# XPU-Forces/mojo_opset

Hardware: AMD Instinct MI355X
Metric: MojoPagedDecodeGQA tokens/s (Llama-3-8B shape, bf16, 1/8 MI355X) (higher is better)
Workload: dtype bf16; 1 GPU; MojoPagedDecodeGQA bf16, B=64, 32q/8kv, head_dim=128, page=16, ctx=4096 uniform, AABB, random block tables (BASELINE configs[1]); per_gpu_batch=64, parallelism=replicas x1 (no collective on this path)

## Files before the change

### mojo_opset_amd/csrc/paged_decode_gqa.hip

```cpp
#include <math.h>
#include <stdlib.h>

#include "common.h"

namespace mojo {

constexpr int DEC_LPT = 16;
constexpr int DEC_TPL = 64 / DEC_LPT;
constexpr int DEC_LOADS = 4;
constexpr int DEC_TILE = DEC_TPL * DEC_LOADS;

template <typename T> struct pack8;
template <> struct pack8<bf16_t> {
  typedef bf16x8 vec;
  typedef bf16x2 pair;
  static __device__ __forceinline__ float dot2(pair a, pair b, float c) {
    return __builtin_amdgcn_fdot2_f32_bf16(a, b, c, false);
  }
};
template <> struct pack8<f16_t> {
  typedef f16x8 vec;
  typedef f16x2 pair;
  static __device__ __forceinline__ float dot2(pair a, pair b, float c) { return __builtin_amdgcn_fdot2(a, b, c, false); }
};
// ... 494 lines not shown
    chunk = ceil_div(len, s2);
    if (chunk < 128) chunk = 128;
    chunk = ceil_div(chunk, DEC_TILE) * DEC_TILE;
  }
  return static_cast<int>(chunk);
}

static int64_t decode_max_len(int64_t page, int64_t max_pages, int64_t hint) {
  const int64_t cap = page * max_pages;
  return (hint > 0 && hint < cap) ? hint : cap;
}

static int64_t decode_swa_cap(int64_t max_len, int64_t local_window, int64_t global_window) {
  int64_t span = global_window > 0 ? ceil_div(global_window, DEC_TILE) * DEC_TILE : 0;
  if (local_window >= 0) span += local_window + DEC_TILE;
  return span < max_len ? span : max_len;
}

static bool decode_use_mfma(int64_t G, int64_t head_dim, int64_t page) {
  const bool pow2 = page > 0 && (page & (page - 1)) == 0;
  if (!pow2 || page < 16 || (head_dim != 64 && head_dim != 128) || G > 16) return false;
  const long long e = MOJO_SWITCH("MOJO_HIP_DECODE_MFMA", -1);
  if (e == 0) return false;
  if (e == 1) return true;
  return G >= 4 || head_dim == 64 || (G != 1 && G != 2);
}

struct DecodeGeom {
  int64_t batch = 0, q_heads = 0, kv_heads = 0, head_dim = 0, page = 0, max_pages = 0, len_hint = 0;
  int64_t local_window = -1, global_window = 0;
  bool kv8 = false;
};

struct DecodePlan {
  bool swa = false;
  bool mfma = false;
  int64_t capacity = 0;
  int64_t max_len = 0;
  int chunk_tokens = 0, n_chunks = 0, fuse_group = 0;
  int hshift = 0, grid_kv_heads = 0, G = 0;
  int64_t slots = 0;
  int64_t bytes = 0;
  int64_t query_bytes = 0;
};

static DecodePlan decode_plan(const DecodeGeom& g) {
  DecodePlan p;
  p.swa = g.local_window >= 0 || g.global_window > 0;
  if (g.batch <= 0 || g.kv_heads <= 0 || g.q_heads <= 0) return p;
  p.capacity = decode_max_len(g.page, g.max_pages, g.len_hint);
  p.max_len = p.swa ? decode_swa_cap(p.capacity, g.local_window, g.global_window) : p.capacity;
  const int64_t heads = g.q_heads / g.kv_heads;
  auto form = [&](int hshift, DecodePlan& f) {
    f.hshift = hshift;
    f.grid_kv_heads = static_cast<int>(g.kv_heads << hshift);
    f.G = static_cast<int>(heads >> hshift);
    f.mfma = !g.kv8 && decode_use_mfma(f.G, g.head_dim, g.page);
    const bool grouped = f.mfma && MOJO_SWITCH("MOJO_HIP_DECODE_GROUPED", 1) != 0 && MOJO_SWITCH("MOJO_HIP_DECODE_FUSE", 1) != 0;
    f.chunk_tokens = decode_chunk_tokens(g.batch, f.grid_kv_heads, p.max_len, grouped);
    f.n_chunks = static_cast<int>(ceil_div(p.max_len > 0 ? p.max_len : 1, f.chunk_tokens));
    f.fuse_group = grouped && f.n_chunks > 8 ? 8 : 0;
    f.slots = g.batch * g.kv_heads * f.n_chunks * heads;
  };
  const bool can_halve = !p.swa && !g.kv8 && heads == 8;
  int hshift = 0;
#ifdef MOJO_HIP_BUILD_EXPERIMENTS
  if (can_halve && MOJO_SWITCH("MOJO_HIP_DECODE_G8_HALVES", 0) == 1) hshift = 1;
#endif
  form(hshift, p);
  const int64_t slot_bytes = (g.head_dim + 2) * static_cast<int64_t>(sizeof(float));
  p.bytes = p.slots * slot_bytes;
  int64_t most = p.slots;
  if (can_halve) {
    DecodePlan other;
    form(1 - hshift, other);
    if (other.slots > most) most = other.slots;
  }
  p.query_bytes = most * slot_bytes + 256;
  return p;
}

template <typename T, bool NT, int MODE, bool SWA>
static void launch_decode_mfma(const DecodeArgs& a, dim3 grid, dim3 block, int G, hipStream_t s) {
  const size_t waves = block.x / 64;
  const size_t lds = (MODE != DEC_SPLIT ? waves * G * (a.dim + 2) * sizeof(float) : 0) + waves * 4096;
  static std::atomic<uint64_t> attr_set{0};
  if (first_call_on_device(attr_set)) {
    (void)hipFuncSetAttribute(reinterpret_cast<const void*>(&decode_mfma_kernel<T, 4, NT, MODE, SWA>), hipFuncAttributeMaxDynamicSharedMemorySize, 160 * 1024);
    (void)hipFuncSetAttribute(reinterpret_cast<const void*>(&decode_mfma_kernel<T, 2, NT, MODE, SWA>), hipFuncAttributeMaxDynamicSharedMemorySize, 160 * 1024);
  }
  if (a.dim == 128) hipLaunchKernelGGL((decode_mfma_kernel<T, 4, NT, MODE, SWA>), grid, block, lds, s, a, G);
  else hipLaunchKernelGGL((decode_mfma_kernel<T, 2, NT, MODE, SWA>), grid, block, lds, s, a, G);
}

template <typename T, bool NT, bool SWA>
static int launch_decode_nt(const DecodeArgs& a, const DecodePlan& p, hipStream_t s) {
  const int64_t batch = a.batch;
  const int G = p.G;
  const bool no_fuse = MOJO_SWITCH("MOJO_HIP_DECODE_FUSE", 1) == 0;
  const bool no_pair = MOJO_SWITCH("MOJO_HIP_DECODE_PAIR", 1) == 0;
  const char* nt_tag = NT ? "nt" : "cached";
  const char* swa_tag = SWA ? ":swa" : "";
  if (p.mfma) {
    if (!SWA && a.n_chunks == 4 && batch >= 2 && batch <= 64 && !no_fuse && !no_pair) {
      launch_decode_mfma<T, NT, DEC_PAIRED, false>(a, dim3(1, static_cast<unsigned>(((batch + 1) / 2) * a.hkv)), dim3(512), G, s);
      MOJO_CHECK_LAUNCH("paged_decode_gqa(mfma, paired)");
      note_launch("decode_mfma:paired:%s%s", nt_tag, swa_tag);
      return MOJO_OK;
    }
    if (a.n_chunks <= 8 && !no_fuse) {
      launch_decode_mfma<T, NT, DEC_FUSED, SWA>(a, dim3(1, static_cast<unsigned>(batch * a.hkv)), dim3(static_cast<unsigned>(64 * a.n_chunks)), G, s);
      MOJO_CHECK_LAUNCH("paged_decode_gqa(mfma, fused)");
      note_launch("decode_mfma:fused:%s%s", nt_tag, swa_tag);
      return MOJO_OK;
    }
    if (a.fuse_group > 0 && !no_fuse) {
      const unsigned n_sub = static_cast<unsigned>((a.n_chunks + a.fuse_group - 1) / a.fuse_group);
      launch_decode_mfma<T, NT, DEC_FUSED, SWA>(a, dim3(n_sub, static_cast<unsigned>(batch * a.hkv)), dim3(static_cast<unsigned>(64 * a.fuse_group)), G, s);
      MOJO_CHECK_LAUNCH("paged_decode_gqa(mfma, grouped)");
      hipLaunchKernelGGL((decode_merge_kernel<T, SWA>), dim3(static_cast<unsigned>(batch * a.hkv), G), dim3(256), 0, s, a, G);
      MOJO_CHECK_LAUNCH("paged_decode_gqa(merge)");
      note_launch("decode_mfma:grouped+merge:%s%s", nt_tag, swa_tag);
      return MOJO_OK;
    }
    launch_decode_mfma<T, NT, DEC_SPLIT, SWA>(a, dim3(static_cast<unsigned>(a.n_chunks), static_cast<unsigned>(batch * a.hkv)), dim3(64), G, s);
    MOJO_CHECK_LAUNCH("paged_decode_gqa(mfma, split)");
    hipLaunchKernelGGL((decode_merge_kernel<T, SWA>), dim3(static_cast<unsigned>(batch * a.hkv), G), dim3(256), 0, s, a, G);
    MOJO_CHECK_LAUNCH("paged_decode_gqa(merge)");
    note_launch("decode_mfma:split+merge:%s%s", nt_tag, swa_tag);
    return MOJO_OK;
  }
  if (!SWA && a.n_chunks == 4 && batch >= 2 && batch <= 64 && a.dim % 4 == 0 && !no_fuse && !no_pair) {
    dim3 grid(1, static_cast<unsigned>(((batch + 1) / 2) * a.hkv));
    const size_t lds = static_cast<size_t>(8) * G * (a.dim + 2) * sizeof(float) + (G >= 8 ? static_cast<size_t>(8) * G * DEC_LPT * 16 : 0);
    switch (G) {
      case 1: hipLaunchKernelGGL((decode_split_kernel<T, 1, NT, DEC_PAIRED, false>), grid, dim3(512), lds, s, a); break;
      case 2: hipLaunchKernelGGL((decode_split_kernel<T, 2, NT, DEC_PAIRED, false>), grid, dim3(512), lds, s, a); break;
      case 4: hipLaunchKernelGGL((decode_split_kernel<T, 4, NT, DEC_PAIRED, false>), grid, dim3(512), lds, s, a); break;
      case 8: hipLaunchKernelGGL((decode_split_kernel<T, 8, NT, DEC_PAIRED, false>), grid, dim3(512), lds, s, a); break;
      default: MOJO_REQUIRE(false, MOJO_EUNSUPPORTED, "paged_decode_gqa: group size %d (supported: 1,2,4,8)", G);
    }
    MOJO_CHECK_LAUNCH("paged_decode_gqa(paired)");
    note_launch("decode_valu:paired:%s%s", nt_tag, swa_tag);
    return MOJO_OK;
  }
  if (a.n_chunks <= 8 && a.dim % 4 == 0 && !no_fuse) {
    dim3 grid(1, static_cast<unsigned>(batch * a.hkv));
    const dim3 block(static_cast<unsigned>(64 * a.n_chunks));
    const size_t lds = static_cast<size_t>(a.n_chunks) * G * (a.dim + 2) * sizeof(float) +
                       (G >= 8 ? static_cast<size_t>(a.n_chunks) * G * DEC_LPT * 16 : 0);
    switch (G) {
      case 1: hipLaunchKernelGGL((decode_split_kernel<T, 1, NT, DEC_FUSED, SWA>), grid, block, lds, s, a); break;
      case 2: hipLaunchKernelGGL((decode_split_kernel<T, 2, NT, DEC_FUSED, SWA>), grid, block, lds, s, a); break;
      case 4: hipLaunchKernelGGL((decode_split_kernel<T, 4, NT, DEC_FUSED, SWA>), grid, block, lds, s, a); break;
      case 8: hipLaunchKernelGGL((decode_split_kernel<T, 8, NT, DEC_FUSED, SWA>), grid, block, lds, s, a); break;
      default: MOJO_REQUIRE(false, MOJO_EUNSUPPORTED, "paged_decode_gqa: group size %d (supported: 1,2,4,8)", G);
    }
    MOJO_CHECK_LAUNCH("paged_decode_gqa(fused)");
    note_launch("decode_valu:fused:%s%s", nt_tag, swa_tag);
    return MOJO_OK;
  }
  dim3 grid(static_cast<unsigned>(a.n_chunks), static_cast<unsigned>(batch * a.hkv));
  switch (G) {
    case 1: hipLaunchKernelGGL((decode_split_kernel<T, 1, NT, DEC_SPLIT, SWA>), grid, dim3(64), 0, s, a); break;
    case 2: hipLaunchKernelGGL((decode_split_kernel<T, 2, NT, DEC_SPLIT, SWA>), grid, dim3(64), 0, s, a); break;
    case 4: hipLaunchKernelGGL((decode_split_kernel<T, 4, NT, DEC_SPLIT, SWA>), grid, dim3(64), 0, s, a); break;
    case 8: hipLaunchKernelGGL((decode_split_kernel<T, 8, NT, DEC_SPLIT, SWA>), grid, dim3(64), 0, s, a); break;
    default: MOJO_REQUIRE(false, MOJO_EUNSUPPORTED, "paged_decode_gqa: group size %d (supported: 1,2,4,8)", G);
  }
  MOJO_CHECK_LAUNCH("paged_decode_gqa(split)");
  hipLaunchKernelGGL((decode_merge_kernel<T, SWA>), dim3(static_cast<unsigned>(batch * a.hkv), G), dim3(256), 0, s, a, G);
  MOJO_CHECK_LAUNCH("paged_decode_gqa(merge)");
  note_launch("decode_valu:split+merge:%s%s", nt_tag, swa_tag);
  return MOJO_OK;
}

template <typename T, bool SWA>
static int launch_decode(const DecodeArgs& a, const DecodePlan& p, hipStream_t s) {
  const bool nt = MOJO_SWITCH("MOJO_HIP_STREAM_NT", -1) != 0;
  return nt ? launch_decode_nt<T, true, SWA>(a, p, s) : launch_decode_nt<T, false, SWA>(a, p, s);
}

}

using namespace mojo;

struct DecodeCall {
  const void *query = nullptr, *key_cache = nullptr, *value_cache = nullptr;
  const int32_t *total_seq_lens = nullptr, *block_tables = nullptr;
  void *out = nullptr, *workspace = nullptr;
  DecodeGeom g;
  int64_t workspace_bytes = 0, block_table_stride = 0, cache_block_stride = 0, cache_head_stride = 0, cache_token_stride = 0;
  float softmax_scale = 0.f;
  int layout_abab = 0, leave_empty_rows = 0, dtype = 0;
  mojo_stream_t stream = nullptr;
};

static int decode_fill_args(DecodeArgs& a, const DecodeCall& c, const DecodePlan& p, const char* op) {
  const DecodeGeom& g = c.g;
  a.q = c.query; a.kc = c.key_cache; a.vc = c.value_cache; a.seq_lens = c.total_seq_lens; a.tables = c.block_tables; a.out = c.out;
  a.hq = static_cast<int>(g.q_heads); a.hkv = p.grid_kv_heads; a.hshift = p.hshift; a.dim = static_cast<int>(g.head_dim);
  a.page = static_cast<int>(g.page); a.max_pages = static_cast<int>(g.max_pages); a.batch = static_cast<int>(g.batch);
  a.page_shift = (g.page & (g.page - 1)) == 0 ? __builtin_ctzll(g.page) : -1;
  a.table_stride = c.block_table_stride; a.c_blk = c.cache_block_stride; a.c_head = c.cache_head_stride; a.c_tok = c.cache_token_stride;
  a.chunk_tokens = p.chunk_tokens; a.n_chunks = p.n_chunks; a.fuse_group = p.fuse_group;
  a.scale_log2 = c.softmax_scale * 1.4426950408889634f; a.abab = c.layout_abab ? 1 : 0; a.leave_empty = c.leave_empty_rows ? 1 : 0;
  MOJO_REQUIRE(c.workspace && c.workspace_bytes >= p.bytes, MOJO_EWORKSPACE, "%s: workspace %lld B < required %lld B", op,
               (long long)c.workspace_bytes, (long long)p.bytes);
  MOJO_REQUIRE(aligned_to(c.workspace, 16), MOJO_EINVAL, "%s: workspace must be 16-byte aligned", op);
  a.ws_acc = static_cast<float*>(c.workspace);
  a.ws_ml = a.ws_acc + p.slots * g.head_dim;
  return MOJO_OK;
}

template <bool SWA>
static int paged_decode_planned(const DecodeCall& c, const DecodePlan& p) {
  const DecodeGeom& g = c.g;
  MOJO_REQUIRE(c.query && c.key_cache && c.value_cache && c.total_seq_lens && c.block_tables && c.out, MOJO_EINVAL,
               "paged_decode_gqa: null pointer");
  MOJO_REQUIRE(g.batch > 0 && g.q_heads > 0 && g.kv_heads > 0 && g.q_heads % g.kv_heads == 0, MOJO_EINVAL,
               "paged_decode_gqa: bad head counts Hq=%lld Hkv=%lld", (long long)g.q_heads, (long long)g.kv_heads);
  MOJO_REQUIRE(c.dtype == MOJO_BF16 || c.dtype == MOJO_F16, MOJO_EUNSUPPORTED,
               "paged_decode_gqa: dtype %d (bf16/fp16 only)", c.dtype);
  MOJO_REQUIRE(g.head_dim % 8 == 0 && g.head_dim >= 8 && g.head_dim <= 8 * DEC_LPT, MOJO_EUNSUPPORTED,
               "paged_decode_gqa: head_dim %lld (multiple of 8, <= %d)", (long long)g.head_dim, 8 * DEC_LPT);
  MOJO_REQUIRE(g.page % DEC_TPL == 0, MOJO_EUNSUPPORTED, "paged_decode_gqa: block_size %lld must be a multiple of %d",
               (long long)g.page, DEC_TPL);
  MOJO_REQUIRE(c.cache_token_stride % 8 == 0 && c.cache_head_stride % 8 == 0 && c.cache_block_stride % 8 == 0 &&
                   aligned_to(c.key_cache, 16) && aligned_to(c.value_cache, 16) && aligned_to(c.query, 16) &&
                   aligned_to(c.out, 16),
               MOJO_EUNSUPPORTED, "paged_decode_gqa: tensors must be 16-byte aligned with 16-byte row strides");
  MOJO_REQUIRE(g.max_pages >= 0 && g.batch * g.kv_heads * 2 <= 65535, MOJO_EUNSUPPORTED,
               "paged_decode_gqa: batch*kv_heads %lld exceeds the grid limit", (long long)(g.batch * g.kv_heads));
  DecodeArgs a;
  if constexpr (SWA) {
    MOJO_REQUIRE(p.capacity < (int64_t{1} << 30) && g.local_window < (int64_t{1} << 30) && g.global_window < (int64_t{1} << 30),
                 MOJO_EUNSUPPORTED, "paged_decode_swa: lengths and windows must stay below 2^30");
    a.swa_cap = static_cast<int>(p.capacity);
    a.local_win = g.local_window >= 0 ? static_cast<int>(g.local_window) : -1;
    a.global_win = g.global_window > 0 ? static_cast<int>(g.global_window) : 0;
  }
  if (const int rc = decode_fill_args(a, c, p, "paged_decode_gqa"); rc != MOJO_OK) return rc;
  hipStream_t s = static_cast<hipStream_t>(c.stream);
  return c.dtype == MOJO_BF16 ? launch_decode<bf16_t, SWA>(a, p, s) : launch_decode<f16_t, SWA>(a, p, s);
}

static int paged_decode(const DecodeCall& c) {
  if (c.g.batch == 0) return MOJO_OK;
  const DecodePlan p = decode_plan(c.g);
  return !p.swa ? paged_decode_planned<false>(c, p) : paged_decode_planned<true>(c, p);
}

extern "C" int64_t mojo_hip_paged_decode_gqa_workspace_bytes(int64_t batch, int64_t q_heads, int64_t kv_heads,
                                                             int64_t head_dim, int64_t block_size,
                                                             int64_t max_blocks_per_seq, int64_t max_seq_len_hint) {
  return decode_plan({batch, q_heads, kv_heads, head_dim, block_size, max_blocks_per_seq, max_seq_len_hint}).query_bytes;
}

extern "C" int64_t mojo_hip_paged_decode_swa_workspace_bytes(int64_t batch, int64_t q_heads, int64_t kv_heads,
                                                             int64_t head_dim, int64_t block_size,
                                                             int64_t max_blocks_per_seq, int64_t max_seq_len_hint,
                                                             int64_t local_window, int64_t global_window) {
  return decode_plan({batch, q_heads, kv_heads, head_dim, block_size, max_blocks_per_seq, max_seq_len_hint, local_window,
                      global_window}).query_bytes;
}

extern "C" int mojo_hip_paged_decode_gqa(const void* query, const void* key_cache, const void* value_cache,
                                         const int32_t* total_seq_lens, const int32_t* block_tables, void* out,
                                         void* workspace, int64_t workspace_bytes, int64_t batch, int64_t q_heads,
                                         int64_t kv_heads, int64_t head_dim, int64_t block_size,
                                         int64_t max_blocks_per_seq, int64_t block_table_stride,
                                         int64_t cache_block_stride, int64_t cache_head_stride,
                                         int64_t cache_token_stride, int64_t max_seq_len_hint, float softmax_scale,
                                         int layout_abab, int leave_empty_rows, int dtype, mojo_stream_t stream) {
  DecodeCall c;
  c.query = query; c.key_cache = key_cache; c.value_cache = value_cache; c.total_seq_lens = total_seq_lens; c.block_tables = block_tables;
  c.out = out; c.workspace = workspace; c.workspace_bytes = workspace_bytes; c.stream = stream;
  c.g = {batch, q_heads, kv_heads, head_dim, block_size, max_blocks_per_seq, max_seq_len_hint};
  c.block_table_stride = block_table_stride; c.cache_block_stride = cache_block_stride; c.cache_head_stride = cache_head_stride;
  c.cache_token_stride = cache_token_stride; c.softmax_scale = softmax_scale; c.layout_abab = layout_abab;
  c.leave_empty_rows = leave_empty_rows; c.dtype = dtype;
  return paged_decode(c);
}

extern "C" int mojo_hip_paged_decode_swa(const void* query, const void* key_cache, const void* value_cache,
                                         const int32_t* total_seq_lens, const int32_t* block_tables, void* out,
                                         void* workspace, int64_t workspace_bytes, int64_t batch, int64_t q_heads,
                                         int64_t kv_heads, int64_t head_dim, int64_t block_size,
                                         int64_t max_blocks_per_seq, int64_t block_table_stride,
                                         int64_t cache_block_stride, int64_t cache_head_stride,
                                         int64_t cache_token_stride, int64_t max_seq_len_hint, float softmax_scale,
                                         int layout_abab, int leave_empty_rows, int dtype, int64_t local_window,
                                         int64_t global_window, mojo_stream_t stream) {
  DecodeCall c;
  c.query = query; c.key_cache = key_cache; c.value_cache = value_cache; c.total_seq_lens = total_seq_lens; c.block_tables = block_tables;
  c.out = out; c.workspace = workspace; c.workspace_bytes = workspace_bytes; c.stream = stream;
  c.g = {batch, q_heads, kv_heads, head_dim, block_size, max_blocks_per_seq, max_seq_len_hint, local_window, global_window};
  c.block_table_stride = block_table_stride; c.cache_block_stride = cache_block_stride; c.cache_head_stride = cache_head_stride;
  c.cache_token_stride = cache_token_stride; c.softmax_scale = softmax_scale; c.layout_abab = layout_abab;
  c.leave_empty_rows = leave_empty_rows; c.dtype = dtype;
  return paged_decode(c);
}

#include "paged_decode_kv8.h"
```

### mojo_opset_amd/csrc/paged_decode_mfma.h

```cpp
#pragma once

namespace mojo {

template <typename T> struct dec_mma;
template <> struct dec_mma<bf16_t> {
  typedef bf16x8 frag8;
  typedef s16x4 frag4;
  static __device__ __forceinline__ f32x4 qk(frag8 a, frag8 b, f32x4 c) { return __builtin_amdgcn_mfma_f32_16x16x32_bf16(a, b, c, 0, 0, 0); }
  static __device__ __forceinline__ f32x4 pv(frag4 a, frag4 b, f32x4 c) { return __builtin_amdgcn_mfma_f32_16x16x16bf16_1k(a, b, c, 0, 0, 0); }
  static __device__ __forceinline__ frag4 pack(float p0, float p1, float p2, float p3) {
    const bf16x4 v = {static_cast<bf16_t>(p0), static_cast<bf16_t>(p1), static_cast<bf16_t>(p2), static_cast<bf16_t>(p3)};
    return __builtin_bit_cast(frag4, v);
  }
  static __device__ __forceinline__ frag4 from_lds(s16x4 v) { return v; }
};
template <> struct dec_mma<f16_t> {
  typedef f16x8 frag8;
  typedef f16x4 frag4;
  static __device__ __forceinline__ f32x4 qk(frag8 a, frag8 b, f32x4 c) { return __builtin_amdgcn_mfma_f32_16x16x32_f16(a, b, c, 0, 0, 0); }
  static __device__ __forceinline__ f32x4 pv(frag4 a, frag4 b, f32x4 c) { return __builtin_amdgcn_mfma_f32_16x16x16f16(a, b, c, 0, 0, 0); }
  static __device__ __forceinline__ frag4 pack(float p0, float p1, float p2, float p3) {
    const f16x4 v = {static_cast<f16_t>(p0), static_cast<f16_t>(p1), static_cast<f16_t>(p2), static_cast<f16_t>(p3)};
    return v;
  }
  static __device__ __forceinline__ frag4 from_lds(s16x4 v) { return __builtin_bit_cast(f16x4, v); }
};

constexpr int DECM_TILE = 16;

template <typename T, int DK , bool NT, int MODE, bool SWA = false >
__global__ __launch_bounds__(MODE != DEC_SPLIT ? 512 : 64) void decode_mfma_kernel(DecodeArgs a, int G) {
  constexpr bool FUSED = MODE != DEC_SPLIT;
  constexpr bool PAIRED = MODE == DEC_PAIRED;
  static_assert(!(SWA && PAIRED), "the paired form takes no window");
  constexpr int D = DK * 32, ND = D / 16;
  constexpr int ROWB = D * 2;
  constexpr int NP = D / 16;
  constexpr int RPB = 8 / NP;
  constexpr int NS = DK == 2 ? 2 : 1;
  constexpr int STEP = DECM_TILE * NS;
  typedef typename pack8<T>::vec V8;
  typedef dec_mma<T> MM;
  const int lane = threadIdx.x & 63;
  const int tl = lane & 15, g4 = lane >> 4;
  const int wave_id = FUSED ? __builtin_amdgcn_readfirstlane(static_cast<int>(threadIdx.x >> 6)) : 0;
  int chunk = FUSED ? static_cast<int>(blockIdx.x) * static_cast<int>(blockDim.x >> 6) + wave_id : static_cast<int>(blockIdx.x);
  int b = blockIdx.y / a.hkv;
  const int kvh = blockIdx.y % a.hkv;

  int seq_len, chunk_tokens;
  DecodeWin win;
  int pb[2] = {0, -1}, plen[2] = {0, 0}, pchunk[2] = {DEC_TILE, DEC_TILE}, n_first = 8;
  if constexpr (PAIRED) {
    const int cap = a.n_chunks * a.chunk_tokens;
    int len = -1;
    if (lane < a.batch) len = a.max_pages > 0 ? max(min(a.seq_lens[lane], cap), 0) : 0;
    int rank = lane;
    if (__ballot(lane < a.batch && len != __builtin_amdgcn_readfirstlane(len)) != 0) {
      rank = 0;
      for (int o = 0; o < a.batch; ++o) {
        const int lo = __builtin_amdgcn_readlane(len, o);
        rank += (lo > len || (lo == len && o < lane)) ? 1 : 0;
      }
    }
    const int p = b;
    const unsigned long long first = __ballot(lane < a.batch && rank == p);
    const unsigned long long second = __ballot(lane < a.batch && rank == a.batch - 1 - p && a.batch - 1 - p > p);
    pb[0] = __builtin_ctzll(first);
    plen[0] = __builtin_amdgcn_readlane(len, pb[0]);
    if (second) {
      pb[1] = __builtin_ctzll(second);
      plen[1] = __builtin_amdgcn_readlane(len, pb[1]);
    }
    const int sum = plen[0] + plen[1];
    n_first = plen[1] <= 0 ? 8 : min(max((8 * plen[0] + sum / 2) / sum, 1), 7);
#pragma unroll
    for (int u = 0; u < 2; ++u) {
      const int n_u = u ? 8 - n_first : n_first;
      int c = n_u > 0 ? (plen[u] + n_u - 1) / n_u : DEC_TILE;
      c = max(c, 128);
      pchunk[u] = ((c + DEC_TILE - 1) / DEC_TILE) * DEC_TILE;
    }
    const int u = wave_id < n_first ? 0 : 1;
    b = pb[u];
    chunk = u ? wave_id - n_first : wave_id;
    seq_len = b >= 0 ? plen[u] : 0;
    chunk_tokens = pchunk[u];
    if (b < 0) b = pb[0];
  } else {
    if constexpr (SWA) seq_len = a.max_pages > 0 ? decode_swa_row(a, b, win) : 0;
    else seq_len = a.max_pages > 0 ? decode_seq_len(a, b) : 0;
    chunk_tokens = decode_seq_chunk(a, seq_len);
  }
  const int tok_begin = chunk * chunk_tokens;
  const bool has_work = seq_len > 0 && tok_begin < seq_len;
  if (!FUSED && !has_work) return;
  const int tok_end = has_work ? min(seq_len, tok_begin + chunk_tokens) : tok_begin + 1;

  const int hq_l = min(tl, G - 1);
  constexpr int NL = D / 64;
  typename MM::frag8 qf[NL][2];

  f32x4 o[ND];
#pragma unroll
  for (int dt = 0; dt < ND; ++dt) o[dt] = f32x4{0.f, 0.f, 0.f, 0.f};
  float m = -INFINITY, l = 0.f;

  const int32_t* table = a.tables + static_cast<int64_t>(b) * a.table_stride;
  int p1 = (tok_end + a.page - 1) / a.page;
  int first_neg = 0x7fffffff;
  if (p1 > a.max_pages) { first_neg = a.max_pages; p1 = a.max_pages; }
  constexpr int SCAN = 4;
  int scan_v[SCAN];
  auto scan_issue = [&](int base) {
#pragma unroll
    for (int u = 0; u < SCAN; ++u) {
      scan_v[u] = table[min(base + u * 64 + lane, p1 - 1)];
    }
  };
  auto scan_reduce = [&](int base) {
#pragma unroll
    for (int u = 0; u < SCAN; ++u) {
      const unsigned long long neg = __ballot(scan_v[u] < 0 && base + u * 64 + lane < p1);
      if (neg && first_neg == 0x7fffffff) first_neg = base + u * 64 + __builtin_ctzll(neg);
    }
  };

  constexpr int CPR = D / 8;
  constexpr int RPI = 64 / CPR;
  constexpr int NV = 16 / RPI;
  const int kt8 = lane & 7, kc8 = lane >> 3;
  const int vr = lane / CPR, vc = lane % CPR;
  const T* kbase = static_cast<const T*>(a.kc) + (kvh >> a.hshift) * a.c_head + kc8 * 8;
  const T* vbase = static_cast<const T*>(a.vc) + (kvh >> a.hshift) * a.c_head + vc * 8;
  const int last_tile = ((tok_end - 1) / DECM_TILE) * DECM_TILE;
  const int last_page = a.max_pages - 1;

  constexpr int IDW = 60;
  static_assert(IDW % (3 * NS) == 0 && IDW + 2 * NS <= 64, "windows change between rounds; a round's requests stay inside one");
  auto id_window = [&](int s_base) -> int {
    int tu = min(tok_begin + DECM_TILE * (s_base + lane), last_tile);
    if constexpr (SWA) tu = decode_swa_real(win, tu);
    return table[min(tu >> a.page_shift, last_page)];
  };
  {
    const int h = decode_head(a, kvh, hq_l, G);
    const T* qp = static_cast<const T*>(a.q) + (static_cast<int64_t>(b) * a.hq + h) * a.dim;
#pragma unroll
    for (int L = 0; L < NL; ++L)
#pragma unroll
      for (int p = 0; p < 2; ++p) qf[L][p] = *reinterpret_cast<const typename MM::frag8*>(qp + (8 * L + 2 * g4 + p) * 8);
  }
  int idw = 0, idn = 0, id_base = 0;
  if (has_work) {
    idw = id_window(0);
    idn = id_window(IDW);
    if constexpr (!SWA) scan_issue(0);
  }
  struct Tile { V8 k[NS][2][NL]; V8 v[NS][NV]; int lp[NS]; };
  auto ld = [&](const T* p) -> V8 {
    if constexpr (NT) return __builtin_nontemporal_load(reinterpret_cast<const V8*>(p));
    else return *reinterpret_cast<const V8*>(p);
  };
  auto load_tile = [&](Tile& t, int t0) {
    const int s0 = __builtin_amdgcn_readfirstlane((t0 - tok_begin) / DECM_TILE) - id_base;
#pragma unroll
    for (int ss = 0; ss < NS; ++ss) {
      int tu = min(t0 + DECM_TILE * ss, last_tile);
      if constexpr (SWA) tu = decode_swa_real(win, tu);
      const int lp = tu >> a.page_shift;
      t.lp[ss] = lp;
      const int phys = max(__builtin_amdgcn_readlane(idw, s0 + ss), 0);
      const int64_t pg = static_cast<int64_t>(phys) * a.c_blk + static_cast<int64_t>(tu - (lp << a.page_shift)) * a.c_tok;
#pragma unroll
      for (int j = 0; j < 2; ++j)
#pragma unroll
        for (int L = 0; L < NL; ++L) t.k[ss][j][L] = ld(kbase + pg + static_cast<int64_t>(8 * j + kt8) * a.c_tok + L * 64);
#pragma unroll
      for (int u = 0; u < NV; ++u) t.v[ss][u] = ld(vbase + pg + static_cast<int64_t>(RPI * u + vr) * a.c_tok);
    }
  };

  extern __shared__ float s_part[];
  const int n_waves = FUSED ? static_cast<int>(blockDim.x >> 6) : 1;
  char* const v_img = reinterpret_cast<char*>(s_part + (FUSED ? n_waves * G * (D + 2) : 0)) + wave_id * (NS * 16 * ROWB);
  const unsigned v_u32 = static_cast<unsigned>(reinterpret_cast<size_t>(v_img));
  unsigned w_off[NV];
#pragma unroll
  for (int u = 0; u < NV; ++u) {
    const int row = RPI * u + vr;
    const int fw = (row / RPB) & (NP - 1);
    w_off[u] = row * ROWB + (((vc >> 1) ^ fw) << 5) + (vc & 1) * 16;
  }
  const int rrow = 4 * g4 + (tl >> 2);
  const int fr = (rrow / RPB) & (NP - 1);
  const unsigned r_base = v_u32 + rrow * ROWB + (tl & 3) * 8;

  auto process = [&](Tile& t, int t0) {
#pragma unroll
    for (int ss = 0; ss < NS; ++ss)
      if (t.lp[ss] >= first_neg) {
        V8 z = {};
#pragma unroll
        for (int j = 0; j < 2; ++j)
#pragma unroll
          for (int L = 0; L < NL; ++L) t.k[ss][j][L] = z;
#pragma unroll
        for (int u = 0; u < NV; ++u) t.v[ss][u] = z;
      }
    const bool full = t0 + STEP <= tok_end;
    int rt[NS];
    bool edge[NS], any_edge = false;
#pragma unroll
    for (int ss = 0; ss < NS; ++ss) {
      rt[ss] = t0 + DECM_TILE * ss;
      edge[ss] = false;
      if constexpr (SWA) {
        rt[ss] = decode_swa_real(win, rt[ss]);
        edge[ss] = decode_swa_edge(win, rt[ss]);
        any_edge = any_edge || edge[ss];
      }
    }
    float x[NS][4];
#pragma unroll
    for (int ss = 0; ss < NS; ++ss) {
      f32x4 c[2][2];
#pragma unroll
      for (int j = 0; j < 2; ++j)
#pragma unroll
        for (int p = 0; p < 2; ++p) {
          c[j][p] = f32x4{0.f, 0.f, 0.f, 0.f};
#pragma unroll
          for (int L = 0; L < NL; ++L) c[j][p] = MM::qk(__builtin_bit_cast(typename MM::frag8, t.k[ss][j][L]), qf[L][p], c[j][p]);
        }
#pragma unroll
      for (int u = 0; u < NV; ++u) {
        const bool vrow_ok = full || (t0 + DECM_TILE * ss + RPI * u + vr) < tok_end;
        V8 z = {};
        *reinterpret_cast<V8*>(v_img + ss * (16 * ROWB) + w_off[u]) = vrow_ok ? t.v[ss][u] : z;
      }
#pragma unroll
      for (int i = 0; i < 4; ++i) {
        const float xa = c[0][1][i], ya = c[1][0][i];
        const auto sw = __builtin_amdgcn_permlane32_swap(__builtin_bit_cast(unsigned, xa), __builtin_bit_cast(unsigned, ya), false, false);
        const float own = lane < 32 ? c[0][0][i] : c[1][1][i];
        const float oth = __builtin_bit_cast(float, lane < 32 ? sw[1] : sw[0]);
        x[ss][i] = (own + oth) * a.scale_log2;
      }
    }
    if (!full || any_edge) {
#pragma unroll
      for (int ss = 0; ss < NS; ++ss)
#pragma unroll
        for (int i = 0; i < 4; ++i) {
          bool ok = t0 + DECM_TILE * ss + 4 * g4 + i < tok_end;
          if constexpr (SWA) ok = ok && (!edge[ss] || decode_swa_vis(win, rt[ss] + 4 * g4 + i));
          if (!ok) x[ss][i] = -INFINITY;
        }
    }
    float mx = fmaxf(fmaxf(x[0][0], x[0][1]), fmaxf(x[0][2], x[0][3]));
#pragma unroll
    for (int ss = 1; ss < NS; ++ss) mx = fmaxf(mx, fmaxf(fmaxf(x[ss][0], x[ss][1]), fmaxf(x[ss][2], x[ss][3])));
    mx = xor_max_16_32(mx);
    float ref = m;
    if (mx - m > 8.0f) ref = mx;
    if (!__all(ref == m)) {
      const float alpha = m == ref ? 1.f : fast_exp2(m - ref);
      l *= alpha;
#pragma unroll
      for (int dt = 0; dt < ND; ++dt) o[dt] *= alpha;
      m = ref;
    }
    const float ms = m == -INFINITY ? 0.f : m;
    typename MM::frag4 pf[NS];
#pragma unroll
    for (int ss = 0; ss < NS; ++ss) {
      float p[4];
#pragma unroll
      for (int i = 0; i < 4; ++i) p[i] = fast_exp2(x[ss][i] - ms);
      l += (p[0] + p[1]) + (p[2] + p[3]);
      pf[ss] = MM::pack(p[0], p[1], p[2], p[3]);
    }
#pragma unroll
    for (int dt = 0; dt < ND; ++dt)
#pragma unroll
      for (int ss = 0; ss < NS; ++ss) {
        const s16x4 vt = __builtin_amdgcn_ds_read_tr16_b64_v4i16(
            reinterpret_cast<__attribute__((address_space(3))) s16x4*>(static_cast<uintptr_t>(r_base + ss * (16 * ROWB) + ((dt ^ fr) << 5))));
        o[dt] = MM::pv(MM::from_lds(vt), pf[ss], o[dt]);
      }
  };

  Tile ta, tb, tc;
  if (has_work) {
    auto scan_rest = [&]() {
      if constexpr (!SWA) {
        scan_reduce(0);
        for (int base = 64 * SCAN; base < p1 && first_neg == 0x7fffffff; base += 64 * SCAN) {
          scan_issue(base);
          scan_reduce(base);
        }
      }
    };
    int t0 = tok_begin;
    load_tile(ta, tok_begin);
    if (tok_begin + 4 * STEP < tok_end) {
      load_tile(tb, tok_begin + STEP);
      scan_rest();
      for (;;) {
        const int t_win = tok_begin + DECM_TILE * (id_base + IDW);
        do {
          load_tile(tc, t0 + 2 * STEP);
          process(ta, t0);
          load_tile(ta, t0 + 3 * STEP);
          process(tb, t0 + STEP);
          load_tile(tb, t0 + 4 * STEP);
          process(tc, t0 + 2 * STEP);
          t0 += 3 * STEP;
        } while (t0 + 4 * STEP < tok_end && t0 < t_win);
        if (t0 < t_win) break;
        asm volatile("v_mov_b32 %0, %1" : "=v"(idw) : "v"(idn));
        id_base += IDW;
        idn = id_window(id_base + IDW);
        if (t0 + 4 * STEP >= tok_end) break;
      }
    } else {
      if (tok_begin + STEP < tok_end) load_tile(tb, tok_begin + STEP);
      scan_rest();
    }
    if (t0 + 2 * STEP < tok_end) load_tile(tc, t0 + 2 * STEP);
    process(ta, t0);
    if (t0 + STEP < tok_end) {
      if (t0 + 3 * STEP < tok_end) load_tile(ta, t0 + 3 * STEP);
      process(tb, t0 + STEP);
      if (t0 + 2 * STEP < tok_end) {
        process(tc, t0 + 2 * STEP);
        if (t0 + 3 * STEP < tok_end) process(ta, t0 + 3 * STEP);
      }
    }
  }

  l = xor_sum_16_32(l);
  const bool head_ok = tl < G;
  if constexpr (FUSED) {
    const int stride = D + 2;
    if (head_ok) {
      float* dst = s_part + (wave_id * G + tl) * stride;
#pragma unroll
      for (int dt = 0; dt < ND; ++dt) *reinterpret_cast<f32x4*>(dst + dt * 16 + 4 * g4) = o[dt];
      if (g4 == 0) { dst[D] = m; dst[D + 1] = l; }
    }
    __syncthreads();
    const int per_head = D / 4;
    typedef typename vec_of<T, 4>::type V4;
    constexpr int UNITS = PAIRED ? 2 : 1;
    for (int item = threadIdx.x; item < UNITS * G * per_head; item += blockDim.x) {
      const int u = item / (G * per_head);
      const int rest = item - u * (G * per_head);
      const int g = rest / per_head, d0 = (rest - g * per_head) * 4;
      int ub, ulen, uchunk, slot0, uwaves;
      if constexpr (PAIRED) {
        ub = pb[u]; ulen = plen[u]; uchunk = pchunk[u];
        slot0 = u ? n_first : 0;
        uwaves = u ? 8 - n_first : n_first;
        if (ub < 0) continue;
      } else {
        ub = b; ulen = seq_len; uchunk = chunk_tokens; slot0 = 0; uwaves = static_cast<int>(blockDim.x >> 6);
      }
      int n_chunks_seq = ulen <= 0 ? 0 : min((ulen + uchunk - 1) / uchunk, uwaves);
      bool partial = false;
      if constexpr (!PAIRED) {
        if (a.fuse_group > 0) {
          const int total = ulen <= 0 ? 0 : (ulen + uchunk - 1) / uchunk;
          partial = total > uwaves;
          n_chunks_seq = min(max(total - static_cast<int>(blockIdx.x) * uwaves, 0), uwaves);
          if (blockIdx.x > 0 && n_chunks_seq == 0) continue;
        }
      }
      if (n_chunks_seq == 0 && a.leave_empty) continue;
      const int h = decode_head(a, kvh, g, G);
      float mx = -INFINITY;
      for (int c = 0; c < n_chunks_seq; ++c) mx = fmaxf(mx, s_part[((slot0 + c) * G + g) * stride + D]);
      f32x4 num = {0.f, 0.f, 0.f, 0.f};
      float den = 0.f;
      for (int c = 0; c < n_chunks_seq; ++c) {
        const float* src = s_part + ((slot0 + c) * G + g) * stride;
        const float w = exp2f(src[D] - mx);
        den = fmaf(w, src[D + 1], den);
        num += f32x4{src[d0], src[d0 + 1], src[d0 + 2], src[d0 + 3]} * w;
      }
      if (partial) {
        const int64_t slot = (static_cast<int64_t>(blockIdx.y) * a.n_chunks + blockIdx.x) * G + g;
        *reinterpret_cast<f32x4*>(a.ws_acc + slot * D + d0) = num;
        if (d0 == 0) { a.ws_ml[slot * 2 + 0] = mx; a.ws_ml[slot * 2 + 1] = den; }
        continue;
      }
      const float inv = n_chunks_seq > 0 ? 1.0f / den : 0.f;
      V4 ov;
#pragma unroll
      for (int e = 0; e < 4; ++e) ov[e] = static_cast<T>(num[e] * inv);
      *reinterpret_cast<V4*>(static_cast<T*>(a.out) + (static_cast<int64_t>(ub) * a.hq + h) * D + d0) = ov;
    }
    return;
  }
  if (!head_ok) return;
  const int n_chunks_seq = (seq_len + chunk_tokens - 1) / chunk_tokens;
  if (n_chunks_seq == 1) {
    const int h = decode_head(a, kvh, tl, G);
    const float inv = 1.0f / l;
    typedef typename vec_of<T, 4>::type V4;
    T* dst = static_cast<T*>(a.out) + (static_cast<int64_t>(b) * a.hq + h) * D + 4 * g4;
#pragma unroll
    for (int dt = 0; dt < ND; ++dt) {
      V4 ov;
#pragma unroll
      for (int e = 0; e < 4; ++e) ov[e] = static_cast<T>(o[dt][e] * inv);
      *reinterpret_cast<V4*>(dst + dt * 16) = ov;
    }
    return;
  }
  const int64_t slot = (static_cast<int64_t>(blockIdx.y) * a.n_chunks + chunk) * G + tl;
  float* dst = a.ws_acc + slot * D + 4 * g4;
#pragma unroll
  for (int dt = 0; dt < ND; ++dt) *reinterpret_cast<f32x4*>(dst + dt * 16) = o[dt];
  if (g4 == 0) {
    a.ws_ml[slot * 2 + 0] = m;
    a.ws_ml[slot * 2 + 1] = l;
  }
}

}
```

Measured before the change: 399,500 tokens/s.

## Restructure decode tail pipeline, force early kernel-arg loads, add waves_per_eu hint

Adds a waves_per_eu(2) occupancy hint to the MFMA decode kernel. It forces all kernel arguments into scalar registers at entry so their loads issue early, and makes the seq_len loads unconditional so they start sooner. The loop tail now breaks before fetching the next id window once the end is near, and it handles the remaining 2, 3 or 4 tiles as explicit schedules with sched barriers. It also adds optional timestamp instrumentation, compiled in only under a debug macro. The risk is higher register pressure and rigid scheduling that may not help the other kernel modes.

```diff
diff --git a/mojo_opset_amd/csrc/paged_decode_gqa.hip b/mojo_opset_amd/csrc/paged_decode_gqa.hip
--- a/mojo_opset_amd/csrc/paged_decode_gqa.hip
+++ b/mojo_opset_amd/csrc/paged_decode_gqa.hip
@@ -820,4 +820,16 @@
   return paged_decode(c);
 }
 
+#ifdef DECODE_DBG_STAMPS
+extern "C" int mojo_hip_debug_decode_stamps(unsigned long long* host_out, int64_t count, int clear) {
+  if (hipDeviceSynchronize() != hipSuccess) return MOJO_ELAUNCH;
+  if (hipMemcpyFromSymbol(host_out, HIP_SYMBOL(mojo::g_dec_stamps), static_cast<size_t>(count) * 8) != hipSuccess) return MOJO_ELAUNCH;
+  if (clear) {
+    void* p = nullptr;
+    if (hipGetSymbolAddress(&p, HIP_SYMBOL(mojo::g_dec_stamps)) != hipSuccess || hipMemset(p, 0, sizeof(mojo::g_dec_stamps)) != hipSuccess) return MOJO_ELAUNCH;
+  }
+  return MOJO_OK;
+}
+#endif
+
 #include "paged_decode_kv8.h"
diff --git a/mojo_opset_amd/csrc/paged_decode_mfma.h b/mojo_opset_amd/csrc/paged_decode_mfma.h
--- a/mojo_opset_amd/csrc/paged_decode_mfma.h
+++ b/mojo_opset_amd/csrc/paged_decode_mfma.h
@@ -28,8 +28,27 @@
 
 constexpr int DECM_TILE = 16;
 
+#ifdef DECODE_DBG_STAMPS
+constexpr int DEC_STAMP_WAVES = 32768, DEC_STAMP_SLOTS = 8;
+__device__ unsigned long long g_dec_stamps[DEC_STAMP_WAVES * DEC_STAMP_SLOTS];
+#define DEC_STAMP(slot)                                                                                       \
+  do {                                                                                                        \
+    __builtin_amdgcn_sched_barrier(0);                                                                        \
+    asm volatile("s_memrealtime %0\n\ts_waitcnt lgkmcnt(0)" : "=s"(dec_stamps[slot])::"memory");              \
+    __builtin_amdgcn_sched_barrier(0);                                                                        \
+  } while (0)
+#define DEC_STAMP_AFTER(slot, cons, dep)                                                                      \
+  do {                                                                                                        \
+    asm volatile("" ::cons(dep));                                                                             \
+    DEC_STAMP(slot);                                                                                          \
+  } while (0)
+#else
+#define DEC_STAMP(slot) do {} while (0)
+#define DEC_STAMP_AFTER(slot, cons, dep) do {} while (0)
+#endif
+
 template <typename T, int DK , bool NT, int MODE, bool SWA = false >
-__global__ __launch_bounds__(MODE != DEC_SPLIT ? 512 : 64) void decode_mfma_kernel(DecodeArgs a, int G) {
+__global__ __launch_bounds__(MODE != DEC_SPLIT ? 512 : 64) __attribute__((amdgpu_waves_per_eu(2))) void decode_mfma_kernel(DecodeArgs a, int G) {
   constexpr bool FUSED = MODE != DEC_SPLIT;
   constexpr bool PAIRED = MODE == DEC_PAIRED;
   static_assert(!(SWA && PAIRED), "the paired form takes no window");
@@ -42,19 +61,30 @@
   typedef typename pack8<T>::vec V8;
   typedef dec_mma<T> MM;
   const int lane = threadIdx.x & 63;
+#ifdef DECODE_DBG_STAMPS
+  unsigned long long dec_stamps[DEC_STAMP_SLOTS] = {};
+#endif
+  DEC_STAMP(0);
+  asm volatile("" ::"s"(a.q), "s"(a.kc), "s"(a.vc), "s"(a.seq_lens), "s"(a.tables), "s"(a.hq), "s"(a.hkv), "s"(a.dim), "s"(a.page),
+               "s"(a.page_shift), "s"(a.max_pages), "s"(a.batch), "s"(a.hshift), "s"(a.table_stride), "s"(a.c_blk), "s"(a.c_head),
+               "s"(a.c_tok), "s"(a.chunk_tokens), "s"(a.n_chunks), "s"(a.abab), "s"(G), "s"(static_cast<int>(blockDim.x)));
+  if constexpr (SWA) asm volatile("" ::"s"(a.swa_cap), "s"(a.local_win), "s"(a.global_win));
+  int n_kvh = a.hkv;
+  asm volatile("" : "+s"(n_kvh) : "s"(a.out), "s"(a.ws_acc), "s"(a.ws_ml), "s"(a.scale_log2), "s"(a.leave_empty), "s"(a.fuse_group));
   const int tl = lane & 15, g4 = lane >> 4;
   const int wave_id = FUSED ? __builtin_amdgcn_readfirstlane(static_cast<int>(threadIdx.x >> 6)) : 0;
   int chunk = FUSED ? static_cast<int>(blockIdx.x) * static_cast<int>(blockDim.x >> 6) + wave_id : static_cast<int>(blockIdx.x);
-  int b = blockIdx.y / a.hkv;
-  const int kvh = blockIdx.y % a.hkv;
+  int b = blockIdx.y / n_kvh;
+  const int kvh = blockIdx.y % n_kvh;
 
   int seq_len, chunk_tokens;
   DecodeWin win;
   int pb[2] = {0, -1}, plen[2] = {0, 0}, pchunk[2] = {DEC_TILE, DEC_TILE}, n_first = 8;
   if constexpr (PAIRED) {
     const int cap = a.n_chunks * a.chunk_tokens;
+    const int raw_len = a.seq_lens[min(lane, a.batch - 1)];
     int len = -1;
-    if (lane < a.batch) len = a.max_pages > 0 ? max(min(a.seq_lens[lane], cap), 0) : 0;
+    if (lane < a.batch) len = a.max_pages > 0 ? max(min(raw_len, cap), 0) : 0;
     int rank = lane;
     if (__ballot(lane < a.batch && len != __builtin_amdgcn_readfirstlane(len)) != 0) {
       rank = 0;
@@ -63,6 +93,7 @@
         rank += (lo > len || (lo == len && o < lane)) ? 1 : 0;
       }
     }
+    DEC_STAMP_AFTER(1, "v", len);
     const int p = b;
     const unsigned long long first = __ballot(lane < a.batch && rank == p);
     const unsigned long long second = __ballot(lane < a.batch && rank == a.batch - 1 - p && a.batch - 1 - p > p);
@@ -88,9 +119,11 @@
     chunk_tokens = pchunk[u];
     if (b < 0) b = pb[0];
   } else {
-    if constexpr (SWA) seq_len = a.max_pages > 0 ? decode_swa_row(a, b, win) : 0;
-    else seq_len = a.max_pages > 0 ? decode_seq_len(a, b) : 0;
+    if constexpr (SWA) seq_len = decode_swa_row(a, b, win);
+    else seq_len = decode_seq_len(a, b);
+    if (a.max_pages <= 0) seq_len = 0;
     chunk_tokens = decode_seq_chunk(a, seq_len);
+    DEC_STAMP_AFTER(1, "s", seq_len);
   }
   const int tok_begin = chunk * chunk_tokens;
   const bool has_work = seq_len > 0 && tok_begin < seq_len;
@@ -303,10 +336,12 @@
       }
     };
     int t0 = tok_begin;
+    DEC_STAMP_AFTER(2, "v", idw);
     load_tile(ta, tok_begin);
     if (tok_begin + 4 * STEP < tok_end) {
       load_tile(tb, tok_begin + STEP);
       scan_rest();
+      DEC_STAMP_AFTER(3, "v", ta.v[NS - 1][NV - 1]);
       for (;;) {
         const int t_win = tok_begin + DECM_TILE * (id_base + IDW);
         do {
@@ -321,23 +356,48 @@
         if (t0 < t_win) break;
         asm volatile("v_mov_b32 %0, %1" : "=v"(idw) : "v"(idn));
         id_base += IDW;
+        if (t0 + 4 * STEP >= tok_end) break;
         idn = id_window(id_base + IDW);
-        if (t0 + 4 * STEP >= tok_end) break;
+      }
+      DEC_STAMP(4);
+      const int left = (tok_end - t0 + STEP - 1) / STEP;
+      auto request = [&](Tile& t, int at) {
+        load_tile(t, at);
+        __builtin_amdgcn_sched_barrier(0);
+      };
+      if (left == 4) {
+        request(tc, t0 + 2 * STEP);
+        process(ta, t0);
+        request(ta, t0 + 3 * STEP);
+        process(tb, t0 + STEP);
+        process(tc, t0 + 2 * STEP);
+        process(ta, t0 + 3 * STEP);
+      } else if (left == 3) {
+        request(tc, t0 + 2 * STEP);
+        process(ta, t0);
+        process(tb, t0 + STEP);
+        process(tc, t0 + 2 * STEP);
+      } else {
+        process(ta, t0);
+        process(tb, t0 + STEP);
       }
     } else {
       if (tok_begin + STEP < tok_end) load_tile(tb, tok_begin + STEP);
       scan_rest();
-    }
-    if (t0 + 2 * STEP < tok_end) load_tile(tc, t0 + 2 * STEP);
-    process(ta, t0);
-    if (t0 + STEP < tok_end) {
-      if (t0 + 3 * STEP < tok_end) load_tile(ta, t0 + 3 * STEP);
-      process(tb, t0 + STEP);
-      if (t0 + 2 * STEP < tok_end) {
-        process(tc, t0 + 2 * STEP);
-        if (t0 + 3 * STEP < tok_end) process(ta, t0 + 3 * STEP);
-      }
-    }
+      DEC_STAMP_AFTER(3, "v", ta.v[NS - 1][NV - 1]);
+      DEC_STAMP(4);
+      if (t0 + 2 * STEP < tok_end) load_tile(tc, t0 + 2 * STEP);
+      process(ta, t0);
+      if (t0 + STEP < tok_end) {
+        if (t0 + 3 * STEP < tok_end) load_tile(ta, t0 + 3 * STEP);
+        process(tb, t0 + STEP);
+        if (t0 + 2 * STEP < tok_end) {
+          process(tc, t0 + 2 * STEP);
+          if (t0 + 3 * STEP < tok_end) process(ta, t0 + 3 * STEP);
+        }
+      }
+    }
+    DEC_STAMP_AFTER(5, "v", o[ND - 1]);
   }
 
   l = xor_sum_16_32(l);
@@ -351,6 +411,7 @@
       if (g4 == 0) { dst[D] = m; dst[D + 1] = l; }
     }
     __syncthreads();
+    DEC_STAMP(6);
     const int per_head = D / 4;
     typedef typename vec_of<T, 4>::type V4;
     constexpr int UNITS = PAIRED ? 2 : 1;
@@ -401,6 +462,14 @@
       for (int e = 0; e < 4; ++e) ov[e] = static_cast<T>(num[e] * inv);
       *reinterpret_cast<V4*>(static_cast<T*>(a.out) + (static_cast<int64_t>(ub) * a.hq + h) * D + d0) = ov;
     }
+#ifdef DECODE_DBG_STAMPS
+    DEC_STAMP(7);
+    const int64_t wave = (static_cast<int64_t>(blockIdx.y) * gridDim.x + blockIdx.x) * 8 + wave_id;
+    if (lane == 0 && wave < DEC_STAMP_WAVES) {
+#pragma unroll
+      for (int i = 0; i < DEC_STAMP_SLOTS; ++i) g_dec_stamps[wave * DEC_STAMP_SLOTS + i] = dec_stamps[i];
+    }
+#endif
     return;
   }
   if (!head_ok) return;
```

Result: no change. 397,700 tokens/s (-0.5%).

## Specialize decode pipeline for hole-free ring and add waves-per-EU hint

Applied to the files above, without the earlier changes.

Splits the main pipelined loop at the first negative page index, so the steady-state tiles skip the per-tile zeroing check and the bounds check through compile-time flags. Tail handling becomes explicit cases, and any region past a hole is processed by a simple unpipelined loop that reloads the id window. Adds an amdgpu_waves_per_eu(2) attribute to steer register allocation, and sched_barriers around process. This adds code size and may limit scheduling freedom across the barriers.

```diff
diff --git a/mojo_opset_amd/csrc/paged_decode_mfma.h b/mojo_opset_amd/csrc/paged_decode_mfma.h
--- a/mojo_opset_amd/csrc/paged_decode_mfma.h
+++ b/mojo_opset_amd/csrc/paged_decode_mfma.h
@@ -27,9 +27,10 @@
 };
 
 constexpr int DECM_TILE = 16;
+template <bool B> struct dec_flag { static constexpr bool value = B; };
 
 template <typename T, int DK , bool NT, int MODE, bool SWA = false >
-__global__ __launch_bounds__(MODE != DEC_SPLIT ? 512 : 64) void decode_mfma_kernel(DecodeArgs a, int G) {
+__global__ __launch_bounds__(MODE != DEC_SPLIT ? 512 : 64) __attribute__((amdgpu_waves_per_eu(2))) void decode_mfma_kernel(DecodeArgs a, int G) {
   constexpr bool FUSED = MODE != DEC_SPLIT;
   constexpr bool PAIRED = MODE == DEC_PAIRED;
   static_assert(!(SWA && PAIRED), "the paired form takes no window");
@@ -196,19 +197,22 @@
   const int fr = (rrow / RPB) & (NP - 1);
   const unsigned r_base = v_u32 + rrow * ROWB + (tl & 3) * 8;
 
-  auto process = [&](Tile& t, int t0) {
-#pragma unroll
-    for (int ss = 0; ss < NS; ++ss)
-      if (t.lp[ss] >= first_neg) {
-        V8 z = {};
-#pragma unroll
-        for (int j = 0; j < 2; ++j)
-#pragma unroll
-          for (int L = 0; L < NL; ++L) t.k[ss][j][L] = z;
-#pragma unroll
-        for (int u = 0; u < NV; ++u) t.v[ss][u] = z;
-      }
-    const bool full = t0 + STEP <= tok_end;
+  auto process = [&](Tile& t, int t0, auto hole_c, auto full_c) {
+    __builtin_amdgcn_sched_barrier(0);
+    if constexpr (decltype(hole_c)::value) {
+#pragma unroll
+      for (int ss = 0; ss < NS; ++ss)
+        if (t.lp[ss] >= first_neg) {
+          V8 z = {};
+#pragma unroll
+          for (int j = 0; j < 2; ++j)
+#pragma unroll
+            for (int L = 0; L < NL; ++L) t.k[ss][j][L] = z;
+#pragma unroll
+          for (int u = 0; u < NV; ++u) t.v[ss][u] = z;
+        }
+    }
+    const bool full = decltype(full_c)::value || t0 + STEP <= tok_end;
     int rt[NS];
     bool edge[NS], any_edge = false;
 #pragma unroll
@@ -302,41 +306,81 @@
         }
       }
     };
+    auto tail_step = [&](Tile& t, int at, auto full_c) {
+      asm volatile("; decode_tail step");
+      process(t, at, dec_flag<false>{}, full_c);
+    };
+    constexpr dec_flag<true> yes{};
+    constexpr dec_flag<false> no{};
+    auto ring_bound = [&]() -> int {
+      if (first_neg == 0x7fffffff) return tok_end;
+      if constexpr (SWA) return tok_begin;
+      const int64_t hole_tok = static_cast<int64_t>(first_neg) << a.page_shift;
+      if (hole_tok >= tok_end) return tok_end;
+      return hole_tok <= tok_begin ? tok_begin : tok_begin + static_cast<int>((hole_tok - tok_begin) / STEP) * STEP;
+    };
     int t0 = tok_begin;
     load_tile(ta, tok_begin);
-    if (tok_begin + 4 * STEP < tok_end) {
+    if (tok_begin + STEP >= tok_end) {
+      scan_rest();
+      if (ring_bound() > tok_begin) {
+        asm volatile("; decode_tail case 1");
+        tail_step(ta, t0, no);
+        t0 += STEP;
+      }
+    } else {
       load_tile(tb, tok_begin + STEP);
       scan_rest();
-      for (;;) {
-        const int t_win = tok_begin + DECM_TILE * (id_base + IDW);
-        do {
+      const int ring_end = ring_bound();
+      if (tok_begin + STEP < ring_end) {
+        if (tok_begin + 4 * STEP < ring_end) {
+          for (;;) {
+            const int t_win = tok_begin + DECM_TILE * (id_base + IDW);
+            do {
+              load_tile(tc, t0 + 2 * STEP);
+              process(ta, t0, no, yes);
+              load_tile(ta, t0 + 3 * STEP);
+              process(tb, t0 + STEP, no, yes);
+              load_tile(tb, t0 + 4 * STEP);
+              process(tc, t0 + 2 * STEP, no, yes);
+              t0 += 3 * STEP;
+            } while (t0 + 4 * STEP < ring_end && t0 < t_win);
+            if (t0 < t_win) break;
+            asm volatile("v_mov_b32 %0, %1" : "=v"(idw) : "v"(idn));
+            id_base += IDW;
+            if (t0 + 4 * STEP >= ring_end) break;
+            idn = id_window(id_base + IDW);
+          }
+        }
+        const int left = (ring_end - t0 + STEP - 1) / STEP;
+        if (left >= 4) {
+          asm volatile("; decode_tail case 4");
           load_tile(tc, t0 + 2 * STEP);
-          process(ta, t0);
+          tail_step(ta, t0, yes);
           load_tile(ta, t0 + 3 * STEP);
-          process(tb, t0 + STEP);
-          load_tile(tb, t0 + 4 * STEP);
-          process(tc, t0 + 2 * STEP);
-          t0 += 3 * STEP;
-        } while (t0 + 4 * STEP < tok_end && t0 < t_win);
-        if (t0 < t_win) break;
-        asm volatile("v_mov_b32 %0, %1" : "=v"(idw) : "v"(idn));
-        id_base += IDW;
-        idn = id_window(id_base + IDW);
-        if (t0 + 4 * STEP >= tok_end) break;
-      }
-    } else {
-      if (tok_begin + STEP < tok_end) load_tile(tb, tok_begin + STEP);
-      scan_rest();
-    }
-    if (t0 + 2 * STEP < tok_end) load_tile(tc, t0 + 2 * STEP);
-    process(ta, t0);
-    if (t0 + STEP < tok_end) {
-      if (t0 + 3 * STEP < tok_end) load_tile(ta, t0 + 3 * STEP);
-      process(tb, t0 + STEP);
-      if (t0 + 2 * STEP < tok_end) {
-        process(tc, t0 + 2 * STEP);
-        if (t0 + 3 * STEP < tok_end) process(ta, t0 + 3 * STEP);
-      }
+          tail_step(tb, t0 + STEP, yes);
+          tail_step(tc, t0 + 2 * STEP, yes);
+          tail_step(ta, t0 + 3 * STEP, no);
+        } else if (left == 3) {
+          asm volatile("; decode_tail case 3");
+          load_tile(tc, t0 + 2 * STEP);
+          tail_step(ta, t0, yes);
+          tail_step(tb, t0 + STEP, yes);
+          tail_step(tc, t0 + 2 * STEP, no);
+        } else {
+          asm volatile("; decode_tail case 2");
+          tail_step(ta, t0, yes);
+          tail_step(tb, t0 + STEP, no);
+        }
+        t0 += left * STEP;
+        asm volatile("" : : "v"(idn));
+      }
+    }
+    for (; t0 < tok_end; t0 += STEP) {
+      id_base = (t0 - tok_begin) / DECM_TILE;
+      idw = id_window(id_base);
+      load_tile(ta, t0);
+      process(ta, t0, yes, no);
     }
   }
 
```

New measurement: 394,900 tokens/s before, 397,400 tokens/s after (median of 2 runs). No clear change (+0.6%).
